# rrwick/Badread

Measured on AMD Instinct MI355X. Metric: simulated bases/sec, higher is better.
Workload: dtype u32

## Files before the change

### badread_amd/csrc/brx_hip.hip

```cpp
#include <hip/hip_runtime.h>
#include <stdarg.h>
#include <stdio.h>
#include <stdlib.h>
#include <string.h>
#include <unistd.h>

#include <algorithm>
#include <vector>

#include "brx_kernels.h"
#include "brx_paf.h"

#define BRX_KEV_MAX 2048

struct brx_ctx {
    int device;
    int n_cu;
    int waves_per_cu;
    BrxDev dev;
    bool has_ref, has_em, has_qm, has_params;
    uint8_t *scratch;
    size_t scratch_bytes;
    size_t scratch_needed, output_needed;
    uint64_t win_bytes;
    uint64_t *h_totals;
    uint8_t *d_totals_alias;
    uint8_t *h_stage, *d_stage;
    size_t stage_bytes;
    uint32_t *h_prog, *d_prog;
    hipEvent_t ev_b[BRX_STAGE_COUNT], ev_e[BRX_STAGE_COUNT];
    float stage_ms[BRX_STAGE_COUNT];
    uint32_t final_launches, mutate_passes;
    uint32_t lanes_cycles;
    int mutate_passes_route;
    uint32_t tail_reads;
    int tb_hmul;
    uint32_t window_misses;
    uint32_t fin_head_reads;
    uint32_t head_reads;
    int wide_stream;
    hipStream_t side2;
    hipEvent_t ev_fork2[2], ev_join2[2], ev_head_mut;
    hipEvent_t ev_fork3, ev_join3[2];
    int fin_spread;
    uint32_t quad_min_reads;
    int fin_lanes;
    uint32_t lanes_min_reads;
    int fin_quad;
    hipStream_t side;
    hipEvent_t ev_fork, ev_join;
    hipEvent_t ev_wait;
    uint64_t *d_clk, *d_phase; uint32_t clk_reads;
    int ktiming;
    hipEvent_t kev_b[BRX_KEV_MAX], kev_e[BRX_KEV_MAX];
    uint8_t kev_kind[BRX_KEV_MAX];
    int kev_n, kev_dropped;
    brx_kernel_stat kstat[BRX_KERN_COUNT];
    int profile;
    bool paf_valid;
    BrxDev paf_dev;
    const RS *paf_rs; const PSeg *paf_segs; uint32_t paf_reads;
    uint8_t *h_paf, *d_paf; size_t paf_bytes;
    char err[512];
};

static int fail(brx_ctx *c, int code, const char *fmt, ...) {
    va_list ap;
    va_start(ap, fmt);
    vsnprintf(c->err, sizeof(c->err), fmt, ap);
    va_end(ap);
    return code;
}

#define HIPCHK(c, call)                                                                              \
    do {                                                                                             \
        hipError_t e_ = (call);                                                                      \
        if (e_ != hipSuccess) return fail((c), BRX_E_HIP, "%s failed: %s", #call, hipGetErrorString(e_)); \
    } while (0)

static bool brx_debug() { static int v = -1; if (v < 0) { const char *e = getenv("BRX_DEBUG"); v = (e && *e && *e != '0') ? 1 : 0; } return v == 1; }
#define DBG(...) do { if (brx_debug()) { fprintf(stderr, "[brx] " __VA_ARGS__); fputc('\n', stderr); fflush(stderr); } } while (0)

#ifndef BRX_GIANT_UNITS
#define BRX_GIANT_UNITS ((uint64_t)64 << 17)
#endif

struct Arena {
    uint8_t *base; size_t cap; size_t used; size_t top;
    void *take(size_t bytes) {
        size_t at = (used + 255) & ~(size_t)255;
        used = at + bytes;
        return used + top <= cap ? base + at : nullptr;
    }
    void *take_top(size_t bytes) {
        if (bytes + top + 256 > cap) { top = cap + 1; return nullptr; }
        const size_t end = (cap - top - bytes) & ~(size_t)255;
        top = cap - end;
        return used + top <= cap ? base + end : nullptr;
    }
    void release_top() { top = 0; }
    size_t room() const { return cap - (top < cap ? top : cap); }
    bool ok() const { return used + top <= cap; }
};

extern "C" const char *brx_version(void) { return "brx-hip 0.1 (gfx950)"; }

static char g_create_err[512] = "";

static void release(brx_ctx *c) {
    if (!c) return;
    for (int i = 0; i < BRX_STAGE_COUNT; ++i) {
        if (c->ev_b[i]) (void)hipEventDestroy(c->ev_b[i]);
        if (c->ev_e[i]) (void)hipEventDestroy(c->ev_e[i]);
    }
    for (int i = 0; i < BRX_KEV_MAX; ++i) {
        if (c->kev_b[i]) (void)hipEventDestroy(c->kev_b[i]);
        if (c->kev_e[i]) (void)hipEventDestroy(c->kev_e[i]);
    }
    if (c->ev_join) (void)hipEventDestroy(c->ev_join);
    if (c->side) (void)hipStreamDestroy(c->side);
    if (c->side2) (void)hipStreamDestroy(c->side2);
    for (int i = 0; i < 2; ++i) { if (c->ev_fork2[i]) (void)hipEventDestroy(c->ev_fork2[i]); if (c->ev_join2[i]) (void)hipEventDestroy(c->ev_join2[i]); }
    if (c->ev_head_mut) (void)hipEventDestroy(c->ev_head_mut);
    if (c->ev_fork3) (void)hipEventDestroy(c->ev_fork3);
    for (int i = 0; i < 2; ++i) if (c->ev_join3[i]) (void)hipEventDestroy(c->ev_join3[i]);
    if (c->ev_fork) (void)hipEventDestroy(c->ev_fork);
    if (c->ev_wait) (void)hipEventDestroy(c->ev_wait);
    if (c->h_totals) (void)hipHostFree(c->h_totals);
    if (c->h_stage) (void)hipHostFree(c->h_stage);
    if (c->h_paf) (void)hipHostFree(c->h_paf);
    free(c);
}

static int create_fail(brx_ctx *c, const char *what, hipError_t e) {
    snprintf(g_create_err, sizeof(g_create_err), "brx_create: %s failed: %s (%d)", what, hipGetErrorString(e), (int)e);
    release(c);
    return BRX_E_HIP;
}

extern "C" int brx_create(int device_id, brx_ctx **out) {
    if (!out) return BRX_E_ARG;
    g_create_err[0] = 0;
    brx_ctx *c = (brx_ctx *)calloc(1, sizeof(brx_ctx));
    if (!c) return BRX_E_ARG;
    c->device = device_id;
    hipError_t e;
    if ((e = hipSetDevice(device_id)) != hipSuccess) return create_fail(c, "hipSetDevice", e);
    int n_cu = 0;
    if ((e = hipDeviceGetAttribute(&n_cu, hipDeviceAttributeMultiprocessorCount, device_id)) != hipSuccess)
        return create_fail(c, "hipDeviceGetAttribute(MultiprocessorCount)", e);
    c->n_cu = n_cu > 0 ? n_cu : 256;
    const char *w = getenv("BRX_WAVES_PER_CU");
    c->waves_per_cu = w ? atoi(w) : 16;
    if (c->waves_per_cu < 1) c->waves_per_cu = 1;
    const char *wb = getenv("BRX_WIN_KB");
    c->win_bytes = (uint64_t)(wb ? atoi(wb) : 512) << 10;
    if ((e = hipHostMalloc((void **)&c->h_totals, 16 * sizeof(uint64_t) + 80 * sizeof(uint32_t), hipHostMallocMapped)) != hipSuccess)
        return create_fail(c, "hipHostMalloc", e);
    c->h_prog = (uint32_t *)(c->h_totals + 16);
    memset(c->h_prog, 0, 80 * sizeof(uint32_t));
    void *dp = nullptr;
    if ((e = hipHostGetDevicePointer(&dp, c->h_totals, 0)) != hipSuccess) return create_fail(c, "hipHostGetDevicePointer", e);
    c->d_totals_alias = (uint8_t *)dp;
    c->d_prog = (uint32_t *)(c->d_totals_alias + 16 * sizeof(uint64_t));
    for (int i = 0; i < BRX_STAGE_COUNT; ++i) {
        if ((e = hipEventCreate(&c->ev_b[i])) != hipSuccess) return create_fail(c, "hipEventCreate", e);
        if ((e = hipEventCreate(&c->ev_e[i])) != hipSuccess) return create_fail(c, "hipEventCreate", e);
    }
    if ((e = hipStreamCreateWithFlags(&c->side, hipStreamNonBlocking)) != hipSuccess) return create_fail(c, "hipStreamCreate", e);
    if ((e = hipStreamCreateWithFlags(&c->side2, hipStreamNonBlocking)) != hipSuccess) return create_fail(c, "hipStreamCreate", e);
    for (int i = 0; i < 2; ++i)
        if ((e = hipEventCreateWithFlags(&c->ev_fork2[i], hipEventDisableTiming)) != hipSuccess ||
            (e = hipEventCreateWithFlags(&c->ev_join2[i], hipEventDisableTiming)) != hipSuccess) return create_fail(c, "hipEventCreate", e);
    if ((e = hipEventCreateWithFlags(&c->ev_head_mut, hipEventDisableTiming)) != hipSuccess) return create_fail(c, "hipEventCreate", e);
    if ((e = hipEventCreateWithFlags(&c->ev_fork3, hipEventDisableTiming)) != hipSuccess ||
        (e = hipEventCreateWithFlags(&c->ev_join3[0], hipEventDisableTiming)) != hipSuccess ||
        (e = hipEventCreateWithFlags(&c->ev_join3[1], hipEventDisableTiming)) != hipSuccess) return create_fail(c, "hipEventCreate", e);
    { const char *v = getenv("BRX_FIN_SPREAD"); c->fin_spread = v ? atoi(v) : 1; }
    { const char *v = getenv("BRX_QUAD_MIN_READS"); c->quad_min_reads = v ? (uint32_t)atoi(v) : 4096u; }
    { const char *v = getenv("BRX_FIN_LANES"); c->fin_lanes = v ? atoi(v) : 1; }
    { const char *v = getenv("BRX_LANES_MIN_READS"); c->lanes_min_reads = v ? (uint32_t)atoi(v) : 2048u; }
    { const char *v = getenv("BRX_FIN_QUAD"); c->fin_quad = v ? (atoi(v) & 1) : 1; }
    { const char *hr = getenv("BRX_HEAD_READS"); c->head_reads = hr ? (uint32_t)atoi(hr) : 1024u; }
    { const char *fh = getenv("BRX_FIN_HEAD_READS"); c->fin_head_reads = fh ? (uint32_t)atoi(fh) : 2048u; }
    { const char *ws = getenv("BRX_WIDE_STREAM"); c->wide_stream = ws ? atoi(ws) : 1; }
    if ((e = hipEventCreateWithFlags(&c->ev_wait, hipEventDisableTiming | hipEventBlockingSync)) != hipSuccess) return create_fail(c, "hipEventCreate", e);
    if ((e = hipEventCreateWithFlags(&c->ev_fork, hipEventDisableTiming)) != hipSuccess) return create_fail(c, "hipEventCreate", e);
    if ((e = hipEventCreateWithFlags(&c->ev_join, hipEventDisableTiming)) != hipSuccess) return create_fail(c, "hipEventCreate", e);
    { const char *pf = getenv("BRX_PROFILE"); c->profile = (pf && atoi(pf)) ? 1 : 0; }
    { const char *tw = getenv("BRX_TB_WINDOW"); c->tb_hmul = tw ? atoi(tw) : 2; }
    { const char *v = getenv("BRX_MUTATE_PASSES"); c->mutate_passes_route = v && atoi(v) != 0; }
    { const char *v = getenv("BRX_LANES_CYCLES"); c->lanes_cycles = v ? (uint32_t)atoi(v) : 96u; }
    { const char *tr = getenv("BRX_TAIL_READS"); c->tail_reads = tr ? (uint32_t)atoi(tr) : 0xFFFFFFFFu; }
    c->err[0] = 0;
    *out = c;
    return BRX_OK;
}

extern "C" void brx_destroy(brx_ctx *c) { release(c); }

extern "C" const char *brx_last_error(const brx_ctx *c) { return c ? c->err : g_create_err; }

extern "C" int brx_set_reference(brx_ctx *c, const brx_reference *r) {
    if (!c || !r) return BRX_E_ARG;
    if (r->n_contigs == 0 || !r->d_packed || !r->d_contigs) return fail(c, BRX_E_ARG, "reference has no contigs");
    c->dev.ref = *r; c->has_ref = true; c->paf_valid = false; return BRX_OK;
}
extern "C" int brx_set_error_model(brx_ctx *c, const brx_error_model *m) {
    if (!c || !m) return BRX_E_ARG;
    if (m->k < 1 || m->k > 16) return fail(c, BRX_E_ARG, "error model k-mer size %d out of range", m->k);
    if (m->type != 0 && (!m->d_rowx || !m->d_altx))
        return fail(c, BRX_E_ARG, "error model without its lookup-order tables (d_rowx, d_altx: include/brx.h)");
    c->dev.em = *m; c->has_em = true; c->paf_valid = false; return BRX_OK;
}
extern "C" int brx_set_qscore_model(brx_ctx *c, const brx_qscore_model *m) {
    if (!c || !m) return BRX_E_ARG;
    if (m->k < 1 || (m->k & 1) == 0 || 2 * m->k + m->gap_bits * (m->k - 1) > 56 || (m->hash_size & (m->hash_size - 1)))
        return fail(c, BRX_E_ARG, "unsupported qscore model geometry");
    c->dev.qm = *m; c->has_qm = true; c->paf_valid = false; return BRX_OK;
}
extern "C" int brx_set_params(brx_ctx *c, const brx_sim_params *p) {
    if (!c || !p) return BRX_E_ARG;
    c->dev.p = *p; c->has_params = true; c->paf_valid = false; return BRX_OK;
}
extern "C" int brx_set_scratch(brx_ctx *c, void *d_scratch, size_t bytes) {
    if (!c) return BRX_E_ARG;
    c->scratch = (uint8_t *)d_scratch; c->scratch_bytes = bytes; c->paf_valid = false; return BRX_OK;
}
extern "C" size_t brx_scratch_needed(const brx_ctx *c) { return c ? c->scratch_needed : 0; }
extern "C" size_t brx_output_needed(const brx_ctx *c) { return c ? c->output_needed : 0; }
extern "C" int brx_last_stage_ms(const brx_ctx *c, float ms[BRX_STAGE_COUNT]) {
    if (!c || !ms) return BRX_E_ARG;
    for (int i = 0; i < BRX_STAGE_COUNT; ++i) ms[i] = c->stage_ms[i];
    return BRX_OK;
}

static int wait_stream(brx_ctx *c, hipStream_t st, const char *what) {
    if (!brx_debug()) {
        HIPCHK(c, hipEventRecord(c->ev_wait, st));
        for (;;) {
            const hipError_t q = hipEventQuery(c->ev_wait);
            if (q == hipSuccess) return BRX_OK;
            if (q != hipErrorNotReady) return fail(c, BRX_E_HIP, "%s: %s", what, hipGetErrorString(q));
            usleep(40);
        }
    }
    const char *w = getenv("BRX_WATCHDOG_S");
    int limit_ms = (w ? atoi(w) : 15) * 1000;
    for (int ms = 0;; ms += 20) {
        hipError_t e = hipStreamQuery(st);
        if (e == hipSuccess) return BRX_OK;
        if (e != hipErrorNotReady) return fail(c, BRX_E_HIP, "%s: %s", what, hipGetErrorString(e));
        if (ms >= limit_ms) {
            fprintf(stderr, "[brx] WATCHDOG: %s stalled; progress words:", what);
            for (int i = 0; i < 64; ++i) fprintf(stderr, "%s%u", (i % 8) ? " " : " | ", c->h_prog[i]);
            fprintf(stderr, "\n"); fflush(stderr);
            _exit(99);
        }
        usleep(20000);
    }
}

extern "C" int brx_last_read_cycles(brx_ctx *c, uint64_t *h_out, uint32_t n_reads) {
    if (!c || !h_out) return BRX_E_ARG;
    if (!c->d_clk || n_reads > c->clk_reads) return fail(c, BRX_E_STATE, "no per-read cycle counters for %u reads", n_reads);
    HIPCHK(c, hipMemcpy(h_out, c->d_clk, (size_t)n_reads * 64, hipMemcpyDeviceToHost));
    return BRX_OK;
}

extern "C" int brx_last_phase_cycles(brx_ctx *c, uint64_t *h_out, uint32_t n_reads) {
    if (!c || !h_out) return BRX_E_ARG;
    if (!c->d_phase || n_reads > c->clk_reads) return fail(c, BRX_E_STATE, "no phase counters for %u reads", n_reads);
    HIPCHK(c, hipMemcpy(h_out, c->d_phase, (size_t)n_reads * 64, hipMemcpyDeviceToHost));
    return BRX_OK;
}
// ... 517 lines not shown
        const uint64_t seq_bytes = c->h_totals[tot_host], ops_bytes = c->h_totals[tot_host + 1];
        uint8_t *seqbuf = (uint8_t *)A.take((size_t)seq_bytes + 64);
        uint8_t *opsbuf = (uint8_t *)A.take((size_t)ops_bytes + 64);
        if (!A.ok()) return scratch_short(c, A.used + A.top + ((size_t)1 << 28));
        {
            KTIMED(BRX_KERN_FIN_JOIN, S.st);
            hipLaunchKernelGGL(k_fin_join, dim3(std::min<uint64_t>(ns, (uint64_t)c->n_cu * 16u)), dim3(64), 0, S.st, dev, rs, order, S.b, S.e,
                               set_counter(S, 0), (uint64_t)(seqbuf - c->scratch), (uint64_t)(opsbuf - c->scratch), Fbuf, repl, pieces, c->scratch,
                               F2buf, c->fin_lanes, c->fin_quad);
        }
        { int rc_ = fetch_rs(S.st); if (rc_) return rc_; }
        { int rcw = wait_stream(c, S.st, "k_fin_join"); if (rcw) return rcw; }
        uint32_t n_quad_set = 0;
        for (uint32_t i = S.b; i < S.e; ++i) { const RS &r = h_rs[h_order[i]]; n_quad_set += (r.n && (r.klass & BRX_KL_QUAD)) ? 1u : 0u; }
        const bool quad_on = n_quad_set >= c->quad_min_reads;
        uint32_t n_lanes_set = 0;
        for (uint32_t i = S.b; i < S.e; ++i) { const RS &r = h_rs[h_order[i]]; n_lanes_set += (r.n && (r.klass & BRX_KL_LANES)) ? 1u : 0u; }
        const bool lanes_on = n_lanes_set >= c->lanes_min_reads;
        for (uint32_t i = S.b; i < S.e; ++i) {
            const RS &r = h_rs[h_order[i]];
            if (!r.n) continue;
            const uint32_t kl = r.klass & 0xFFFFu;
            S.bases_by_class[((r.klass & BRX_KL_LANES) && lanes_on) ? 5 : ((r.klass & BRX_KL_QUAD) && quad_on) ? (brx_quad_words(r.m, r.n, r.ub) == 2 ? 7 : 6) : kl <= 1 ? 0 : kl == 2 ? 1 : kl == 4 ? 2 : 3] += r.n;
            S.bases_by_class[4] += r.n;
        }
        return launch_final_phase(S, 0);
    };

    auto finish_final = [&](FinalSet &S) -> int {
        if (S.e == S.b) return BRX_OK;
        uint32_t *h_ctr = reinterpret_cast<uint32_t *>(c->h_totals + 8);
        if (S.wide != S.st) { int rcw = wait_stream(c, S.wide, "final stage, widest class"); if (rcw) return rcw; }
        { int rc_ = to_host(c, S.st, h_ctr, set_counter(S, 1), 4); if (rc_) return rc_; }
        { int rcw = wait_stream(c, S.st, S.id ? "final stage (bulk)" : "final stage (head)"); if (rcw) return rcw; }
        const uint32_t misses = h_ctr[0];
        c->window_misses += misses;
        if (!misses) return BRX_OK;
        { int rc_ = fetch_rs(S.st); if (rc_) return rc_; }
        { int rcw_ = wait_stream(c, S.st, "final stage, misses"); if (rcw_) return rcw_; }
        int rcp = launch_final_phase(S, 1);
        if (rcp) return rcp;
        if (S.wide != S.st) { int rcw = wait_stream(c, S.wide, "final stage, second phase, widest class"); if (rcw) return rcw; }
        return wait_stream(c, S.st, "final stage, second phase");
    };

    { int rc_ = to_host(c, st, h_order, order, (size_t)n_reads * 4); if (rc_) return rc_; }
    HIPCHK(c, hipMemsetAsync(msv, 0, (size_t)n_reads * sizeof(MS), st));
    HIPCHK(c, hipMemsetAsync(pq, 0, (size_t)n_reads * sizeof(PQ), st));
    HIPCHK(c, hipMemsetAsync(mctr, 0, 8 * MC_WORDS * sizeof(uint32_t), st));
    HIPCHK(c, hipMemsetAsync(lane_cls, 0, 2 * MC_WORDS * BRX_CLS_STRIDE * sizeof(uint32_t), st));
    {
        uint32_t *h_ctr = reinterpret_cast<uint32_t *>(c->h_totals + 8);
        memset(h_ctr, 0, 2 * MC_WORDS * sizeof(uint32_t));
        h_ctr[MC_OUT] = n_mb;
        h_ctr[MC_WORDS + MC_OUT] = n_mh;
        { int rc_ = to_device(c, st, mctr + 2 * MC_WORDS, h_ctr, MC_WORDS * sizeof(uint32_t)); if (rc_) return rc_; }
        { int rc_ = to_device(c, st, mctr + 4 * MC_WORDS, h_ctr + MC_WORDS, MC_WORDS * sizeof(uint32_t)); if (rc_) return rc_; }
        { int rcw_ = wait_stream(c, st, "mutate counters"); if (rcw_) return rcw_; }
    }
    auto launch_run = [&](hipStream_t s, uint32_t count, const uint32_t *act_in, const uint32_t *n_in, uint32_t *ctr, const MutAux *aux) {
        KTIMED(BRX_KERN_MUTATE_RUN, s);
#define BRX_LAUNCH_RUN(PROF)                                                                                                        \
        hipLaunchKernelGGL((k_mutate_seg<PROF, BRX_SEG_WPS>), dim3(std::min(count, side_waves)), dim3(64), 0, s, dev, rs, msv, act_in, n_in,   \
                           ctr, aux, Fbuf, repl, F2buf, Cbuf)
        if (c->profile) BRX_LAUNCH_RUN(true); else BRX_LAUNCH_RUN(false);
#undef BRX_LAUNCH_RUN
    };
    HIPCHK(c, hipEventRecord(c->ev_b[BRX_STAGE_MUTATE], st));
    if (n_mh) {
        if (n_mb) {
            HIPCHK(c, hipEventRecord(c->ev_fork, st));
            HIPCHK(c, hipStreamWaitEvent(s_head, c->ev_fork, 0));
        }
        launch_run(s_head, n_mh, order, mctr + 4 * MC_WORDS + MC_OUT, mctr + 6 * MC_WORDS, aux_dev + 1);
        if (n_mb) HIPCHK(c, hipEventRecord(c->ev_head_mut, s_head));
        c->mutate_passes = 1;
    }
    int rc2 = BRX_OK;
    if (n_mb && !c->mutate_passes_route) {
        const uint32_t post_waves = std::min<uint64_t>(n_mb, (uint64_t)c->n_cu * 32u);
        const uint32_t groups = (n_mb + 63u) / 64u;
        {
            KTIMED(BRX_KERN_MUT_POST, st);
            hipLaunchKernelGGL((k_mut_fill<BRX_POST_U>), dim3(post_waves), dim3(64), 0, st, dev, rs, pq, order + n_mh, n_mb, Fbuf, F2buf, Cbuf, sv_a, sv_z);
        }
        uint32_t *left_ctr = mctr + MC_OUT;
        {
            KTIMED(BRX_KERN_MUTATE_SEG, st);
            if (c->profile)
                hipLaunchKernelGGL((k_mut_lanes<BRX_POST_U, true>), dim3(std::min(groups, lane_waves)), dim3(64), 0, st, dev, rs, msv, pq, order + n_mh, n_mb, h_aux[0],
                                   Fbuf, repl, F2buf, Cbuf, sv_a, sv_z, lane_tb, c->lanes_cycles ? c->lanes_cycles : 0xFFFFFFFFu, active_a, left_ctr);
            else
                hipLaunchKernelGGL((k_mut_lanes<BRX_POST_U, false>), dim3(std::min(groups, lane_waves)), dim3(64), 0, st, dev, rs, msv, pq, order + n_mh, n_mb, h_aux[0],
                                   Fbuf, repl, F2buf, Cbuf, sv_a, sv_z, lane_tb, c->lanes_cycles ? c->lanes_cycles : 0xFFFFFFFFu, active_a, left_ctr);
        }
        if (c->lanes_cycles) {
            launch_run(st, std::min<uint32_t>(n_mb, 8192u), active_a, left_ctr, mctr, aux_dev);
            c->mutate_passes += 1;
        }
        {
            KTIMED(BRX_KERN_MUT_POST, st);
            hipLaunchKernelGGL(k_mut_epilogue, dim3(post_waves), dim3(64), 0, st, dev, rs, msv, order + n_mh, n_mb, h_aux[0], Fbuf, repl);
        }
        c->mutate_passes += 1;
    } else if (n_mb) {
        const uint32_t post_waves = std::min<uint64_t>(n_mb, (uint64_t)c->n_cu * 32u);
        uint32_t *h_ctr = reinterpret_cast<uint32_t *>(c->h_totals + 8);
        uint32_t *legacy_ctr = mctr + 3 * MC_WORDS;
        const uint32_t *n_in = mctr + 2 * MC_WORDS + MC_OUT;
        const uint32_t *act_in = order + n_mh;
        uint32_t n_up = n_mb, pass = 0;
        const uint32_t tail_reads = tail_eff;
        auto read_counts = [&](uint32_t *ctr) -> int {
            { int rc_ = to_host(c, st, h_ctr, ctr, MC_WORDS * sizeof(uint32_t)); if (rc_) return rc_; }
            return wait_stream(c, st, "mutate pass");
        };
        auto poll_head = [&]() -> int {
            if (!n_mh || sets[0].launched || hipEventQuery(c->ev_head_mut) != hipSuccess) return BRX_OK;
            return start_final(sets[0]);
        };
        for (; n_up > 0 && pass < (1u << 20); ++pass) {
            uint32_t *ctr = mctr + (pass & 1u) * MC_WORDS;
            uint32_t *act_out = (pass & 1u) ? active_b : active_a;
            if (n_up <= tail_reads) {
                if (c->ktiming) {
                    std::vector<uint32_t> h_act(n_up);
                    HIPCHK(c, hipMemcpyAsync(h_act.data(), act_in, (size_t)n_up * 4, hipMemcpyDeviceToHost, st));
                    { int rc_ = fetch_rs(st); if (rc_) return rc_; }
                    HIPCHK(c, hipStreamSynchronize(st));
                    for (uint32_t x : h_act) if (x < n_reads) tail_bases += h_rs[x].n;
                }
                launch_run(st, n_up, act_in, n_in, ctr, aux_dev);
                rc2 = read_counts(ctr);
                if (rc2) return rc2;
                n_up = h_ctr[MC_OUT];
                ++pass;
                break;
            }
            if (pass == 0) {
                KTIMED(BRX_KERN_MUT_POST, st);
                hipLaunchKernelGGL((k_mut_post<BRX_POST_U>), dim3(std::min(post_waves, n_up)), dim3(64), 0, st, dev, rs, msv, pq, act_in, n_in,
                                   h_aux[0], Fbuf, repl, F2buf, Cbuf, sv_a, sv_z);
            }
            {
                KTIMED(BRX_KERN_MUTATE_SEG, st);
                hipLaunchKernelGGL(k_mut_apply, dim3((n_up + 63u) / 64u), dim3(64), 0, st, dev, rs, msv, pq, act_in, n_in, sv_a, sv_z, repl, Cbuf);
            }
            {
                KTIMED(BRX_KERN_MUT_POST, st);
                hipLaunchKernelGGL((k_mut_post<BRX_POST_U>), dim3(std::min(post_waves, n_up)), dim3(64), 0, st, dev, rs, msv, pq, act_in, n_in,
                                   h_aux[0], Fbuf, repl, F2buf, Cbuf, sv_a, sv_z);
                hipLaunchKernelGGL(k_pass_lists, dim3((n_up + 63u) / 64u), dim3(64), 0, st, msv, act_in, n_in, act_out, ctr,
                                   lane_cls + (pass & 1u) * MC_WORDS * BRX_CLS_STRIDE, h_aux[0], n_reads);
            }
            {
                KTIMED(BRX_KERN_WIN_LANE, st);
                hipLaunchKernelGGL(k_win_lane, dim3(std::min(lane_waves, (n_up + 63) / 64 + BRX_LANE_CLASSES)), dim3(64), 0, st, msv, req_easy,
                                   lane_cls + (pass & 1u) * MC_WORDS * BRX_CLS_STRIDE, n_reads, winbuf, lane_tb);
            }
            {
                KTIMED(BRX_KERN_WIN_WAVE, st);
                hipLaunchKernelGGL(k_win_wave, dim3(std::min(std::min(side_waves, 512u), n_up)), dim3(64), 0, st, msv, req_hard, ctr + MC_HARD,
                                   ctr + 5, winbuf, win, (uint64_t)c->win_bytes, counters + 1, mctr + ((pass + 1) & 1u) * MC_WORDS,
                                   lane_cls + ((pass + 1) & 1u) * MC_WORDS * BRX_CLS_STRIDE);
            }
            if (n_up <= 4 * std::min<uint32_t>(tail_reads, 48u) || n_up <= tail_reads + 64 || (pass & 3u) == 3u) {
                rc2 = read_counts(ctr);
                if (rc2) return rc2;
                n_up = h_ctr[MC_OUT];
                rc2 = poll_head();
                if (rc2) return rc2;
            }
            n_in = ctr + MC_OUT;
            act_in = act_out;
        }
        c->mutate_passes += pass;
        if (n_up > 0) return fail(c, BRX_E_INTERNAL, "mutate pipeline did not converge after %u passes", pass);
        {
            KTIMED(BRX_KERN_MUT_POST, st);
            hipLaunchKernelGGL(k_mut_epilogue, dim3(std::min(post_waves, n_mb)), dim3(64), 0, st, dev, rs, msv, order + n_mh, n_mb, h_aux[0], Fbuf, repl);
        }
    }
    if (!n_mh) {
        uint32_t *h_ctr = reinterpret_cast<uint32_t *>(c->h_totals + 8);
        uint32_t *legacy_ctr = mctr + 3 * MC_WORDS;
        { int rc_ = to_host(c, st, h_ctr, legacy_ctr, 2 * sizeof(uint32_t)); if (rc_) return rc_; }
        { int rcw = wait_stream(c, st, "mutate stage"); if (rcw) return rcw; }
        if (h_ctr[0] > 0)
            hipLaunchKernelGGL(k_mutate, dim3(std::min(side_waves, h_ctr[0])), dim3(64), 0, st, dev, rs, req_legacy, legacy_ctr,
                               legacy_ctr + 1, Fbuf, repl, win, (uint64_t)c->win_bytes, counters + 1, clk);
        legacy_handled = true;
        if (n_head && n_bulk) {
            HIPCHK(c, hipEventRecord(c->ev_fork, st));
            HIPCHK(c, hipStreamWaitEvent(s_head, c->ev_fork, 0));
        }
    }
    HIPCHK(c, hipEventRecord(c->ev_e[BRX_STAGE_MUTATE], st));
    HIPCHK(c, hipEventRecord(c->ev_b[BRX_STAGE_SCAN], st));
    HIPCHK(c, hipEventRecord(c->ev_e[BRX_STAGE_SCAN], st));
    HIPCHK(c, hipEventRecord(c->ev_b[BRX_STAGE_FINAL], st));
    if (!sets[0].launched) { rc2 = start_final(sets[0]); if (rc2) return rc2; }
    rc2 = start_final(sets[1]); if (rc2) return rc2;
    rc2 = finish_final(sets[0]); if (rc2) return rc2;
    rc2 = finish_final(sets[1]); if (rc2) return rc2;
    if (n_head && n_bulk) {
        HIPCHK(c, hipEventRecord(c->ev_join, s_head));
        HIPCHK(c, hipStreamWaitEvent(st, c->ev_join, 0));
    }
    HIPCHK(c, hipEventRecord(c->ev_e[BRX_STAGE_FINAL], st));
    HIPCHK(c, hipEventRecord(c->ev_b[BRX_STAGE_EMIT], st));

    {
        KTIMED(BRX_KERN_EMIT, st);
        hipLaunchKernelGGL(k_recsize, dim3(nb64), dim3(64), 0, st, dev, rs, pieces);
        hipLaunchKernelGGL(k_scan_rec, dim3(1), dim3(64), 0, st, n_reads, rs, totals);
    }
    rc = read_totals(c, st, totals, 6);
    if (rc) return rc;
    const uint64_t rec_bytes = c->h_totals[5];
    if (rec_bytes > out_cap) {
        c->output_needed = rec_bytes;
        return fail(c, BRX_E_OUTPUT, "output buffer too small: need %llu bytes", (unsigned long long)rec_bytes);
    }
    {
        KTIMED(BRX_KERN_EMIT, st);
        hipLaunchKernelGGL(k_emit, dim3(n_reads), dim3(64), 0, st, dev, rs, pieces, c->scratch, d_out);
        hipLaunchKernelGGL(k_stats, dim3(nb64), dim3(64), 0, st, dev, rs, d_stats);
    }
    HIPCHK(c, hipEventRecord(c->ev_e[BRX_STAGE_EMIT], st));
    { int rcw = wait_stream(c, st, "final stage / k_emit"); if (rcw) return rcw; }
    HIPCHK(c, hipGetLastError());
    for (int i = 0; i < BRX_STAGE_COUNT; ++i) {
        float ms = 0.f;
        if (i != BRX_STAGE_ALIGN1 && i != BRX_STAGE_QSCORE) (void)hipEventElapsedTime(&ms, c->ev_b[i], c->ev_e[i]);
        c->stage_ms[i] = ms;
    }
    if (c->ktiming) {
        if (n_head && n_bulk) HIPCHK(c, hipStreamSynchronize(c->side));
        if (sets[0].wide_forked) HIPCHK(c, hipStreamSynchronize(c->side2));
        for (int i = 0; i < c->kev_n; ++i) {
            float ms = 0.f;
            if (hipEventElapsedTime(&ms, c->kev_b[i], c->kev_e[i]) != hipSuccess) continue;
            c->kstat[c->kev_kind[i]].launches += 1;
            c->kstat[c->kev_kind[i]].ms += ms;
        }
        uint64_t all = 0, head_b = 0;
        for (uint32_t i = 0; i < n_reads; ++i) { all += h_rs[h_order[i]].n; if (i < n_head) head_b += h_rs[h_order[i]].n; }
        if (n_mb && !c->mutate_passes_route && c->lanes_cycles) {
            uint32_t left = 0;
            if (hipMemcpy(&left, mctr + MC_OUT, 4, hipMemcpyDeviceToHost) == hipSuccess && left <= n_reads && left) {
                std::vector<uint32_t> h_left(left);
                if (hipMemcpy(h_left.data(), active_a, (size_t)left * 4, hipMemcpyDeviceToHost) == hipSuccess)
                    for (uint32_t x : h_left) if (x < n_reads) tail_bases += h_rs[x].n;
            }
        }
        double by_class[4] = {0.0, 0.0, 0.0, 0.0};
        for (const FinalSet &S_ : sets) for (int k_ = 0; k_ < 4; ++k_) by_class[k_] += (double)S_.bases_by_class[k_];
        c->kstat[BRX_KERN_PLAN].bases = c->kstat[BRX_KERN_BUILD].bases = c->kstat[BRX_KERN_FIN_JOIN].bases =
            c->kstat[BRX_KERN_FIN_QSCORE].bases = c->kstat[BRX_KERN_EMIT].bases = (double)all;
        c->kstat[BRX_KERN_MUTATE_RUN].bases = (double)(head_b + tail_bases);
        c->kstat[BRX_KERN_MUTATE_SEG].bases = c->kstat[BRX_KERN_MUT_POST].bases = c->kstat[BRX_KERN_WIN_LANE].bases = c->kstat[BRX_KERN_WIN_WAVE].bases = (double)(all - head_b);
        c->kstat[BRX_KERN_FIN_ALIGN1].bases = by_class[0]; c->kstat[BRX_KERN_FIN_ALIGN2].bases = by_class[1];
        c->kstat[BRX_KERN_FIN_ALIGN4].bases = by_class[2]; c->kstat[BRX_KERN_FIN_ALIGN16].bases = by_class[3];
// ... 215 lines not shown
```

### badread_amd/csrc/brx_passes.h

```cpp
#ifndef BRX_PASSES_H
#define BRX_PASSES_H

#ifndef BRX_SV_CAP
#define BRX_SV_CAP 256u
#endif
#ifndef BRX_SV_STOCK
#define BRX_SV_STOCK 56u
#endif
#ifndef BRX_POST_U
#define BRX_POST_U 2
#endif
static_assert((BRX_SV_CAP & (BRX_SV_CAP - 1u)) == 0u && BRX_SV_CAP >= 64u * BRX_POST_U + BRX_SV_STOCK, "ring: a power of two with room for a trip");

struct PQ { uint32_t head, tail, next_t, pad; };

enum { MP_HUNGRY = 4,
       MP_PARK = 5,
       MP_FINISH = 6 };

__device__ __forceinline__ uint32_t brx_loop_cap32(uint32_t n) {
    const uint64_t cap = 100ull * (uint64_t)n;
    return cap > 0xFFFFFF00ull ? 0xFFFFFF00u : (uint32_t)cap;
}

// ... 157 lines not shown
    while (have < stock && have + 64u * (uint32_t)U <= ring_cap && q.next_t < cap) {
        uint32_t ip[U]; BrxProp pr[U]; bool sv[U];
#pragma unroll
        for (int u = 0; u < U; ++u) {
            const uint32_t t = q.next_t + 64u * (uint32_t)u + (uint32_t)lane;
            sv[u] = false; ip[u] = 0u; pr[u].x = pr[u].y = pr[u].z = 0u;
            if (t < cap) sv[u] = brx_propose_iter(d, d.first_read + r, t, max_i1, f2g, oddg, coded, F, &ip[u], &pr[u]);
        }
#pragma unroll
        for (int u = 0; u < U; ++u) {
            const unsigned long long m = __ballot(sv[u]);
            if (sv[u]) {
                const uint32_t slot = (q.tail + (uint32_t)__popcll(m & ((1ull << lane) - 1ull))) % ring_cap;
                ra[slot] = make_uint4(q.next_t + 64u * (uint32_t)u + (uint32_t)lane, ip[u], pr[u].x, pr[u].y);
                rz[slot] = pr[u].z;
            }
            const uint32_t cnt = (uint32_t)__popcll(m);
            q.tail += cnt; have += cnt;
        }
        const uint32_t room = cap - q.next_t;
        q.next_t += room < 64u * (uint32_t)U ? room : 64u * (uint32_t)U;
    }
    if (lane == 0 && (q.tail != tail0 || q.next_t != next0)) { pq[r].tail = q.tail; pq[r].next_t = q.next_t; }
}

template <int U>
__global__ void __launch_bounds__(64, 8) k_mut_post(BrxDev d, RS *rs, MS *msv, PQ *pq, const uint32_t *active_in, const uint32_t *n_in_ptr,
                                                     const MutAux aux, const uint8_t *Fbuf, uint32_t *repl,
                                                     const uint32_t *F2buf, const uint32_t *Cbuf, uint4 *sv_a, uint32_t *sv_z) {
    const int lane = lane_id();
    const brx_error_model &em = d.em;
    const int k = em.k;
    const uint32_t n_in = uni(*n_in_ptr);
    for (uint32_t qi = blockIdx.x; qi < n_in; qi += gridDim.x) {
        const uint32_t r = uni(active_in[qi]);
        const RS s = rs[r];
        if (s.n == 0) continue;
        const uint64_t t_begin = __builtin_amdgcn_s_memtime();
        MS ms = msv[r];
        const uint32_t n = s.n;
        const uint8_t *F = Fbuf + s.F_off;
        uint32_t *rp = repl + s.F_off;
        uint64_t *ck = aux.clk + (uint64_t)r * 8;
        bool goes_on = false;
        if (ms.phase == (uint32_t)MP_PARK) {
            uint32_t a = 0, b = n;
            if (n > BRX_ALIGN_SIZE) {
                uint32_t ww[4];
                brx_draw4(d.seed, d.first_read + r, BRX_ST_WIN, (uint64_t)ms.nalign, ww);
                a = (uint32_t)brx_mulhi64(((uint64_t)ww[1] << 32) | ww[0], (uint64_t)n - BRX_ALIGN_SIZE + 1);
                b = a + BRX_ALIGN_SIZE;
            }
            uint32_t cost = 0;
            uint8_t *qb = aux.winbuf + (uint64_t)r * BRX_WIN_STRIDE, *tbuf = qb + BRX_WIN_Q;
            bool odd = false;
            const uint32_t tl = wave_park<true>(em, F, rp, a, b, qb, tbuf, BRX_WIN_TMAX, &cost, &odd, reinterpret_cast<uint32_t *>(qb + BRX_WIN_PLANES));
            const uint32_t ql = b - a;
            uint32_t klass = MC_LEGACY;
            int band_blocks_of = 0;
            if (tl <= BRX_WIN_TMAX) {
                const BrxGeom g = brx_make_geom((int)ql, (int)tl, (int)cost);
                const int band_blocks = (g.dhi - g.dlo) / 32 + 2;
                band_blocks_of = band_blocks;
                const bool easy = !odd && g.G == 1 && tl <= BRX_LANE_TMAX && ql > 0 && tl > 0 && band_blocks <= BRX_LANE_W;
                klass = easy ? MC_EASY : MC_HARD;
            }
            if (lane == 0) {
                MS *o = &msv[r];
                o->nalign = ms.nalign + 1u;
                o->phase = klass == MC_LEGACY ? 3u : 1u;
                o->win_a = a; o->win_b = b; o->tl = tl; o->cost = cost; o->res_ncols = 0; o->res_nmatch = 0;
                o->passes = ms.passes + 1u;
                o->win_kind = klass | (brx_lane_class(band_blocks_of) << 8);
            }
            goes_on = klass != MC_LEGACY;
        } else if (ms.phase == (uint32_t)MP_FINISH) {
        } else goes_on = true;
        if (goes_on) brx_propose_ahead<U>(d, r, rs, pq, Fbuf, F2buf, Cbuf, sv_a + (size_t)r * BRX_SV_CAP, sv_z + (size_t)r * BRX_SV_CAP, BRX_SV_CAP, BRX_SV_STOCK);
        if (lane == 0) ck[0] += __builtin_amdgcn_s_memtime() - t_begin;
    }
}

__global__ void __launch_bounds__(64, 8) k_mut_epilogue(BrxDev d, RS *rs, MS *msv, const uint32_t *list, uint32_t n_list, const MutAux aux,
                                                         const uint8_t *Fbuf, const uint32_t *repl) {
    const int lane = lane_id();
    const brx_error_model &em = d.em;
    const int k = em.k;
    for (uint32_t qi = blockIdx.x; qi < n_list; qi += gridDim.x) {
        const uint32_t r = uni(list[qi]);
        if (uni(msv[r].phase) != (uint32_t)MP_FINISH) continue;
        const RS s = rs[r];
        const MS ms = msv[r];
        const uint32_t n = s.n;
        const uint8_t *F = Fbuf + s.F_off;
        const uint32_t *rp = repl + s.F_off;
        uint32_t cost = 0;
        const uint32_t m = wave_join(em, F, rp, 0, n, nullptr, &cost);
        uint32_t st = 0, et = 0;
        if (lane < k) { st = rep_len(rp[lane]); et = rep_len(rp[n - k + lane]); }
        st = wave_sum(st); et = wave_sum(et);
        if (lane == 0) {
            RS *o = &rs[r];
            o->status = s.status | ms.status; o->m = m; o->ub = cost; o->start_trim = st; o->end_trim = et;
            o->loops = (uint32_t)ms.round_loops; o->changes = ms.change; o->naligns = ms.nalign;
            o->units = 0;
            msv[r].phase = 2u;
            aux.clk[(uint64_t)r * 8 + 1] = ms.passes;
        }
    }
}

__global__ void __launch_bounds__(64) k_pass_lists(const MS *msv, const uint32_t *active_in, const uint32_t *n_in_ptr, uint32_t *active_out,
                                                    uint32_t *ctr, uint32_t *lane_cls, const MutAux aux, uint32_t n_reads) {
    const uint32_t idx = blockIdx.x * 64u + (uint32_t)lane_id();
    const bool in = idx < *n_in_ptr;
    const uint32_t r = in ? active_in[idx] : 0u;
    const uint32_t phase = in ? msv[r].phase : 0xFFu, kind = in ? msv[r].win_kind : 0u;
    const bool parked = phase == 1u;
    const uint32_t klass = kind & 0xFFu, cls = kind >> 8;
    {
        const bool p = parked || phase == (uint32_t)MP_HUNGRY;
        const uint32_t at = atomicAdd(&ctr[MC_OUT], p ? 1u : 0u);
        if (p) active_out[at] = r;
    }
#pragma unroll
    for (uint32_t cc = 0; cc < (uint32_t)BRX_LANE_CLASSES; ++cc) {
        const bool p = parked && klass == (uint32_t)MC_EASY && cls == cc;
        if (__ballot(p) == 0ull) continue;
        const uint32_t at = atomicAdd(&lane_cls[cc * BRX_CLS_STRIDE], p ? 1u : 0u);
        if (p) aux.req_easy[(size_t)cc * n_reads + at] = r;
    }
    {
        const bool p = parked && klass == (uint32_t)MC_HARD;
        if (__ballot(p) != 0ull) {
            const uint32_t at = atomicAdd(&ctr[MC_HARD], p ? 1u : 0u);
            if (p) aux.req_hard[at] = r;
        }
    }
    {
        const bool p = phase == 3u;
        if (__ballot(p) != 0ull) {
            const uint32_t at = atomicAdd(aux.legacy_ctr, p ? 1u : 0u);
            if (p) aux.req_legacy[at] = r;
        }
    }
}

#ifndef BRX_LANES_MAX_WAVES
#define BRX_LANES_MAX_WAVES 1024u
#endif
#ifndef BRX_RING_SHIFT
#define BRX_RING_SHIFT 3
#define BRX_RING_MIN 128u
#endif
__device__ __forceinline__ uint64_t brx_ring_base(const RS *rs, uint32_t r) { return (rs[r].F_off >> BRX_RING_SHIFT) + (uint64_t)BRX_RING_MIN * (uint64_t)r; }
__device__ __forceinline__ uint32_t brx_ring_cap(const RS *rs, uint32_t r) { return (rs[r].n >> BRX_RING_SHIFT) + BRX_RING_MIN; }

__device__ __forceinline__ uint32_t brx_ring_want(uint32_t n, double target) {
    const double need = (double)n * (1.0 - target);
    if (need < 0.5) return 0u;
    const double t = target > 0.05 ? target : 0.05;
    const double s = 0.9 * need / (t * brx_sqrt(t)) + 32.0;
    return s > 4.0e9 ? 0xF0000000u : (uint32_t)s;
}

template <int U>
__global__ void __launch_bounds__(64, 8) k_mut_fill(BrxDev d, const RS *rs, PQ *pq, const uint32_t *list, uint32_t n_list, const uint8_t *Fbuf,
                                                     const uint32_t *F2buf, const uint32_t *Cbuf, uint4 *sv_a, uint32_t *sv_z) {
    for (uint32_t qi = blockIdx.x; qi < n_list; qi += gridDim.x) {
        const uint32_t r = uni(list[qi]);
        const uint32_t n = uni(rs[r].n);
        if (n == 0u) continue;
        const uint64_t base = uni(brx_ring_base(rs, r));
        const uint32_t cap = uni(brx_ring_cap(rs, r));
        uint32_t want = brx_ring_want(n, rs[r].target);
        want = uni(want);
        const uint32_t room = cap - 64u * (uint32_t)U;
        brx_propose_ahead<U>(d, r, rs, pq, Fbuf, F2buf, Cbuf, sv_a + base, sv_z + base, cap, want < room ? want : room);
    }
}

__device__ inline void brx_lane_park(const brx_error_model &em, const uint8_t *__restrict__ F, const uint32_t *__restrict__ rp,
                                     const uint32_t *__restrict__ cm, const uint32_t a, const uint32_t b,
                                     uint32_t *__restrict__ pl, uint32_t *tl_out, uint32_t *cost_out, bool *odd_out) {
    constexpr uint32_t TW = BRX_LANE_TMAX / 32;
    uint32_t tl = 0, cost = 0;
    bool odd = false;
    uint32_t tlo = 0, thi = 0;
    const uint32_t ql = b - a;
    auto append = [&](uint32_t lo, uint32_t hi, uint32_t nb) {
        const uint32_t sh = tl & 31u;
        if (tl < BRX_LANE_TMAX) {
            tlo |= lo << sh; thi |= hi << sh;
            if (sh + nb >= 32u) {
                pl[64u + (tl >> 5)] = tlo; pl[64u + TW + (tl >> 5)] = thi;
                tlo = sh ? lo >> (32u - sh) : 0u; thi = sh ? hi >> (32u - sh) : 0u;
            }
        }
        tl += nb;
    };
    for (uint32_t x0 = 0; x0 < ql; x0 += 32u) {
        const uint32_t p0 = a + x0;
        const uint32_t nv = ql - x0 < 32u ? ql - x0 : 32u;
        const BrxB16 f0 = *reinterpret_cast<const BrxB16 *>(F + p0);
        const BrxB16 f1 = *reinterpret_cast<const BrxB16 *>(F + p0 + 16u);
        const uint32_t m0 = cm[p0 >> 5], m1 = cm[(p0 >> 5) + 1u];
        const uint32_t live = nv >= 32u ? 0xFFFFFFFFu : (1u << nv) - 1u;
        uint32_t changed = (uint32_t)(((((uint64_t)m1) << 32) | (uint64_t)m0) >> (p0 & 31u)) & live;
        const uint32_t fw[8] = {f0.x, f0.y, f0.z, f0.w, f1.x, f1.y, f1.z, f1.w};
        uint32_t qlo = 0, qhi = 0, oddbits = 0;
#pragma unroll
        for (int q = 0; q < 8; ++q) {
            qlo |= brx_byte_bits(fw[q], 0) << (4 * q); qhi |= brx_byte_bits(fw[q], 1) << (4 * q);
            oddbits |= (fw[q] & 0xFCFCFCFCu) ? (0xFu << (4 * q)) : 0u;
        }
        qlo &= live; qhi &= live;
        if (oddbits & live) {
            for (uint32_t i = 0; i < nv; ++i) odd |= (((fw[i >> 2] >> (8u * (i & 3u))) & 0xFCu) != 0u);
        }
        pl[x0 >> 5] = qlo; pl[32u + (x0 >> 5)] = qhi;
        uint32_t cur = 0;
        while (changed) {
            const uint32_t c = (uint32_t)__ffs((int)changed) - 1u;
            changed &= changed - 1u;
            if (c > cur) { const uint32_t g = c - cur, mk = (1u << g) - 1u; append((qlo >> cur) & mk, (qhi >> cur) & mk, g); }
            const uint32_t w = rp[p0 + c];
            const uint32_t sym = (fw[c >> 2] >> (8u * (c & 3u))) & 0xFFu;
            const uint32_t len = (w >> 24) & 0x7Fu;
            bool has = false;
            for (uint32_t y = 0; y < len; ++y) {
                const uint32_t ch = (uint32_t)rep_char(em, w, y);
                odd |= ch > 3u; has |= ch == sym;
                append(ch & 1u, (ch >> 1) & 1u, 1u);
            }
            cost += len < 2u ? 1u : len - (has ? 1u : 0u);
            cur = c + 1u;
        }
        if (nv > cur) { const uint32_t g = nv - cur, mk = g >= 32u ? 0xFFFFFFFFu : (1u << g) - 1u; append((qlo >> cur) & mk, (qhi >> cur) & mk, g); }
    }
    if (tl <= BRX_LANE_TMAX && (tl & 31u) != 0u) { pl[64u + (tl >> 5)] = tlo; pl[64u + TW + (tl >> 5)] = thi; }
    *tl_out = tl; *cost_out = cost; *odd_out = odd;
}

#define BRX_LPH(i) do { if constexpr (PROFILE) { const uint64_t now_ = __builtin_amdgcn_s_memtime(); lph[i] += now_ - lph_t; lph_t = now_; } } while (0)
template <int U, bool PROFILE = false>
__global__ void __launch_bounds__(64, 4) k_mut_lanes(BrxDev d, RS *rs, MS *msv, PQ *pq, const uint32_t *list, uint32_t n_list, const MutAux aux,
                                                      const uint8_t *Fbuf, uint32_t *repl, const uint32_t *F2buf, uint32_t *Cbuf,
                                                      uint4 *sv_a, uint32_t *sv_z, uint2 *tbw_base, uint32_t max_cycles,
                                                      uint32_t *left_list, uint32_t *left_ctr) {
    const int lane = lane_id();
    const brx_error_model &em = d.em;
    uint2 *tbw = tbw_base + (uint64_t)blockIdx.x * BRX_LANE_TB_UNITS;
    uint2 *tb_wave = reinterpret_cast<uint2 *>(aux.scr_base + (uint64_t)blockIdx.x * aux.scr_bytes);
    for (uint32_t grp = blockIdx.x; 64u * grp < n_list; grp += gridDim.x) {
        const uint32_t idx = 64u * grp + (uint32_t)lane;
        const uint32_t r = idx < n_list ? list[idx] : 0u;
        bool active = idx < n_list && rs[r].n != 0u;
        const uint64_t base = active ? brx_ring_base(rs, r) : 0ull;
        const uint32_t cap = active ? brx_ring_cap(rs, r) : 1u;
        const uint32_t n = active ? rs[r].n : 0u;
        const uint8_t *F = Fbuf + (active ? rs[r].F_off : 0ull);
// ... 109 lines not shown
```

Measured before the change: 3.246 billion.

## Add LDS-cached threshold prefilter for mutation fill and sparse epilogue cost

Adds a block-wide fill kernel that copies a 16-bit per-row threshold table into LDS. It prefilters candidate mutation draws cheaply with a ballot, queues survivors per wave in shared memory, and runs the full propose only on compacted candidates. This is meant to cut global table lookups and wasted propose work on the many draws that get rejected. The epilogue also changes: it computes length and cost by walking only the positions flagged in the change bitmap, instead of a full wave_join over the read. Risks are LDS pressure (32KB of table per block) and correctness, which depends on the prefilter matching propose_iter's acceptance test and on the bitmap covering every changed position.

Result: slower. 3.108 billion (-4.2%).

```diff
diff --git a/badread_amd/csrc/brx_hip.hip b/badread_amd/csrc/brx_hip.hip
--- a/badread_amd/csrc/brx_hip.hip
+++ b/badread_amd/csrc/brx_hip.hip
@@ -32,6 +32,7 @@
     float stage_ms[BRX_STAGE_COUNT];
     uint32_t final_launches, mutate_passes;
     uint32_t lanes_cycles;
+    int fill_lds;
     int mutate_passes_route;
     uint32_t tail_reads;
     int tb_hmul;
@@ -191,6 +192,7 @@
     { const char *tw = getenv("BRX_TB_WINDOW"); c->tb_hmul = tw ? atoi(tw) : 2; }
     { const char *v = getenv("BRX_MUTATE_PASSES"); c->mutate_passes_route = v && atoi(v) != 0; }
     { const char *v = getenv("BRX_LANES_CYCLES"); c->lanes_cycles = v ? (uint32_t)atoi(v) : 96u; }
+    { const char *v = getenv("BRX_FILL_LDS"); c->fill_lds = v ? (atoi(v) != 0) : 1; }
     { const char *tr = getenv("BRX_TAIL_READS"); c->tail_reads = tr ? (uint32_t)atoi(tr) : 0xFFFFFFFFu; }
     c->err[0] = 0;
     *out = c;
@@ -874,7 +876,12 @@
         const uint32_t groups = (n_mb + 63u) / 64u;
         {
             KTIMED(BRX_KERN_MUT_POST, st);
-            hipLaunchKernelGGL((k_mut_fill<BRX_POST_U>), dim3(post_waves), dim3(64), 0, st, dev, rs, pq, order + n_mh, n_mb, Fbuf, F2buf, Cbuf, sv_a, sv_z);
+            const brx_error_model &em = c->dev.em;
+            if (c->fill_lds && em.type != 0 && em.k <= 7 && em.n_rows == (1u << (2 * em.k))) {
+                const uint32_t fill_blocks = std::min<uint64_t>((n_mb + BRX_FILL_WAVES - 1u) / BRX_FILL_WAVES, (uint64_t)c->n_cu * 4u);
+                hipLaunchKernelGGL((k_mut_fill_lds<BRX_POST_U>), dim3(fill_blocks), dim3(64 * BRX_FILL_WAVES), 0, st, dev, rs, pq, order + n_mh, n_mb, Fbuf, F2buf, Cbuf, sv_a, sv_z);
+            } else
+                hipLaunchKernelGGL((k_mut_fill<BRX_POST_U>), dim3(post_waves), dim3(64), 0, st, dev, rs, pq, order + n_mh, n_mb, Fbuf, F2buf, Cbuf, sv_a, sv_z);
         }
         uint32_t *left_ctr = mctr + MC_OUT;
         {
@@ -892,7 +899,7 @@
         }
         {
             KTIMED(BRX_KERN_MUT_POST, st);
-            hipLaunchKernelGGL(k_mut_epilogue, dim3(post_waves), dim3(64), 0, st, dev, rs, msv, order + n_mh, n_mb, h_aux[0], Fbuf, repl);
+            hipLaunchKernelGGL(k_mut_epilogue, dim3(post_waves), dim3(64), 0, st, dev, rs, msv, order + n_mh, n_mb, h_aux[0], Fbuf, repl, Cbuf);
         }
         c->mutate_passes += 1;
     } else if (n_mb) {
@@ -970,7 +977,7 @@
         if (n_up > 0) return fail(c, BRX_E_INTERNAL, "mutate pipeline did not converge after %u passes", pass);
         {
             KTIMED(BRX_KERN_MUT_POST, st);
-            hipLaunchKernelGGL(k_mut_epilogue, dim3(std::min(post_waves, n_mb)), dim3(64), 0, st, dev, rs, msv, order + n_mh, n_mb, h_aux[0], Fbuf, repl);
+            hipLaunchKernelGGL(k_mut_epilogue, dim3(std::min(post_waves, n_mb)), dim3(64), 0, st, dev, rs, msv, order + n_mh, n_mb, h_aux[0], Fbuf, repl, Cbuf);
         }
     }
     if (!n_mh) {
diff --git a/badread_amd/csrc/brx_passes.h b/badread_amd/csrc/brx_passes.h
--- a/badread_amd/csrc/brx_passes.h
+++ b/badread_amd/csrc/brx_passes.h
@@ -263,7 +263,7 @@
 }
 
 __global__ void __launch_bounds__(64, 8) k_mut_epilogue(BrxDev d, RS *rs, MS *msv, const uint32_t *list, uint32_t n_list, const MutAux aux,
-                                                         const uint8_t *Fbuf, const uint32_t *repl) {
+                                                         const uint8_t *Fbuf, const uint32_t *repl, const uint32_t *Cbuf) {
     const int lane = lane_id();
     const brx_error_model &em = d.em;
     const int k = em.k;
@@ -275,8 +275,22 @@
         const uint32_t n = s.n;
         const uint8_t *F = Fbuf + s.F_off;
         const uint32_t *rp = repl + s.F_off;
-        uint32_t cost = 0;
-        const uint32_t m = wave_join(em, F, rp, 0, n, nullptr, &cost);
+        const uint32_t *cm = Cbuf + (s.F_off >> 4);
+        const uint32_t nwc = (n + 31u) >> 5;
+        uint32_t delta = 0, c = 0;
+        for (uint32_t w0 = 0; w0 < nwc; w0 += 64u) {
+            const uint32_t wi = w0 + (uint32_t)lane;
+            uint32_t bits = wi < nwc ? cm[wi] : 0u;
+            while (bits) {
+                const uint32_t p = 32u * wi + (uint32_t)__ffs((int)bits) - 1u;
+                bits &= bits - 1u;
+                const uint32_t w = rp[p];
+                delta += ((w >> 24) & 0x7Fu) - 1u;
+                c += rep_cost(em, w, F[p]);
+            }
+        }
+        const uint32_t m = n + wave_sum(delta);
+        const uint32_t cost = wave_sum(c);
         uint32_t st = 0, et = 0;
         if (lane < k) { st = rep_len(rp[lane]); et = rep_len(rp[n - k + lane]); }
         st = wave_sum(st); et = wave_sum(et);
@@ -358,6 +372,99 @@
         want = uni(want);
         const uint32_t room = cap - 64u * (uint32_t)U;
         brx_propose_ahead<U>(d, r, rs, pq, Fbuf, F2buf, Cbuf, sv_a + base, sv_z + base, cap, want < room ? want : room);
+    }
+}
+
+#define BRX_FILL_ROWS 16384u
+#define BRX_FILL_WAVES 8u
+#define BRX_FILL_QUEUE 128u
+template <int U>
+__global__ void __launch_bounds__(64 * BRX_FILL_WAVES, 8) k_mut_fill_lds(BrxDev d, const RS *rs, PQ *pq, const uint32_t *list, uint32_t n_list, const uint8_t *Fbuf,
+                                                                          const uint32_t *F2buf, const uint32_t *Cbuf, uint4 *sv_a, uint32_t *sv_z) {
+    __shared__ uint16_t thr16[BRX_FILL_ROWS];
+    __shared__ uint32_t fill_q[BRX_FILL_WAVES * BRX_FILL_QUEUE];
+    const brx_error_model &em = d.em;
+    for (uint32_t x = threadIdx.x; x < em.n_rows; x += 64u * BRX_FILL_WAVES) thr16[x] = (uint16_t)(em.d_rowx[2u * x] >> 16);
+    __syncthreads();
+    const int lane = lane_id();
+    const uint32_t wave = uni((uint32_t)threadIdx.x >> 6);
+    const unsigned long long below = (1ull << lane) - 1ull;
+    const int k = em.k;
+    uint32_t *fq = fill_q + wave * BRX_FILL_QUEUE;
+    for (uint32_t qi = blockIdx.x * BRX_FILL_WAVES + wave; qi < n_list; qi += gridDim.x * BRX_FILL_WAVES) {
+        const uint32_t r = uni(list[qi]);
+        const uint32_t n = uni(rs[r].n);
+        if (n == 0u) continue;
+        const uint64_t base = uni(brx_ring_base(rs, r));
+        const uint32_t ring_cap = uni(brx_ring_cap(rs, r));
+        uint32_t want = brx_ring_want(n, rs[r].target);
+        want = uni(want);
+        const uint32_t room = ring_cap - 64u * (uint32_t)U;
+        const uint32_t stock = want < room ? want : room;
+        uint4 *ra = sv_a + base;
+        uint32_t *rz = sv_z + base;
+        const uint64_t F_off = uni(rs[r].F_off);
+        const uint8_t *F = Fbuf + F_off;
+        PQ q = pq[r];
+        q.head = uni(q.head); q.tail = uni(q.tail); q.next_t = uni(q.next_t);
+        const uint32_t tail0 = q.tail, next0 = q.next_t;
+        const uint32_t cap = brx_loop_cap32(n);
+        const uint32_t max_i1 = n - (uint32_t)k;
+        const uint32_t *f2g = F2buf + (F_off >> 4);
+        const uint32_t nw2 = (n + 15u) >> 4, nwc = (n + 31u) >> 5;
+        const bool coded = uni(f2g[nw2] == 0u);
+        const uint32_t *oddg = Cbuf + (F_off >> 4) + nwc;
+        const uint64_t read = d.first_read + r;
+        uint32_t have = q.tail - q.head, nq = 0u, qh = 0u;
+        for (;;) {
+            const bool scan = q.next_t < cap && have + nq < stock && have + nq + 64u <= ring_cap;
+            if (scan) {
+                const uint32_t t = q.next_t + (uint32_t)lane;
+                bool cand = false;
+                if (t < cap) {
+                    uint32_t w[4];
+                    brx_draw4(d.seed, read, BRX_ST_MUT, (uint64_t)t, w);
+                    const uint32_t ipos = (uint32_t)brx_mulhi64(((uint64_t)w[1] << 32) | w[0], (uint64_t)max_i1);
+                    const uint32_t wi = ipos >> 4, sh = 2u * (ipos & 15u);
+                    const uint32_t w0 = f2g[wi], w1 = f2g[wi + 1u];
+                    const uint32_t row = (uint32_t)(((((uint64_t)w0 << 32) | (uint64_t)w1) << sh) >> (64 - 2 * k));
+                    bool bad = false;
+                    if (!coded) {
+                        const uint64_t both = (((uint64_t)oddg[(ipos >> 5) + 1u] << 32) | (uint64_t)oddg[ipos >> 5]) >> (ipos & 31u);
+                        bad = (both & ((1ull << k) - 1ull)) != 0ull;
+                    }
+                    cand = bad || (w[2] >> 16) >= (uint32_t)thr16[row];
+                }
+                const unsigned long long m = __ballot(cand);
+                if (cand) fq[(qh + nq + (uint32_t)__popcll(m & below)) & (BRX_FILL_QUEUE - 1u)] = t;
+                nq += (uint32_t)__popcll(m);
+                const uint32_t left = cap - q.next_t;
+                q.next_t += left < 64u ? left : 64u;
+            }
+            if (nq >= 64u || (!scan && nq != 0u)) {
+                __builtin_amdgcn_wave_barrier();
+                const uint32_t take = nq < 64u ? nq : 64u;
+                uint32_t t = 0u, ip = 0u;
+                BrxProp pr; pr.x = pr.y = pr.z = 0u;
+                bool sv = false;
+                if ((uint32_t)lane < take) {
+                    t = fq[(qh + (uint32_t)lane) & (BRX_FILL_QUEUE - 1u)];
+                    sv = brx_propose_iter(d, read, t, max_i1, f2g, oddg, coded, F, &ip, &pr);
+                }
+                const unsigned long long m = __ballot(sv);
+                if (sv) {
+                    const uint32_t slot = (q.tail + (uint32_t)__popcll(m & below)) % ring_cap;
+                    ra[slot] = make_uint4(t, ip, pr.x, pr.y);
+                    rz[slot] = pr.z;
+                }
+                const uint32_t cnt = (uint32_t)__popcll(m);
+                q.tail += cnt; have += cnt;
+                qh = (qh + take) & (BRX_FILL_QUEUE - 1u); nq -= take;
+                continue;
+            }
+            if (!scan) break;
+        }
+        if (lane == 0 && (q.tail != tail0 || q.next_t != next0)) { pq[r].tail = q.tail; pq[r].next_t = q.next_t; }
     }
 }
 
```
